# chenxuhao/GraphMiner

Hardware: AMD Instinct MI355X
Metric: million edges processed/sec + total match count (higher is better)
Workload: dtype int32 (vertex ids, offsets; uint64 counts); 1 GPU; tc: triangle counting, LiveJournal stand-in; graph=rmat_s22_ef10_seed42, nv=4194304, ne_sym=81171116, tasks=40585558, max_degree=777, parallelism=task-chunk round-robin x1, replicated CSR

## Files before the change

graphminer_amd/csrc/gm_launch.hip:

```cpp
#include "gm_launch.h"

using namespace gm;

__host__ __device__ static inline int finalize_math(int mode, unsigned long long base, const unsigned long long *c, unsigned long long *out) {
  if (mode == FIN_MOTIF3) {
    out[0] = c[2] - c[0];
    out[1] = c[1];
  } else if (mode == FIN_MOTIF3_FORMULA) {
    out[0] = base - 3ull * c[0];
    out[1] = c[0];
  } else if (mode == FIN_RAW4) {
    out[0] = c[0]; out[1] = c[1]; out[2] = c[2]; out[3] = c[3];
  } else if (mode == FIN_HALF_SIGNED) {
    out[0] = (unsigned long long)((long long)c[0] >> 1);
  } else {
    out[0] = c[0];
  }
  return mode == FIN_RAW4 ? 4 : (mode == FIN_MOTIF3 || mode == FIN_MOTIF3_FORMULA) ? 2 : 1;
}

__global__ void finalize_kernel(int mode, unsigned long long base, const unsigned long long *__restrict__ c,
                                unsigned long long *__restrict__ out) {
  if (threadIdx.x != 0 || blockIdx.x != 0) return;
  finalize_math(mode, base, c, out);
// ... 163 lines not shown
      if (const int rc_t = ensure_tasklists(g)) return rc_t;
    }
  }
  if (pl.support && !pl.sup_part && !pl.wtri && !g->diamond.sup) HIP_TRY(g->diamond.sup.alloc(sizeof(unsigned) * (size_t)std::max<long long>(g->ne, 1)));
  if (pl.support && !pl.sup_part && !pl.wtri && world == 1 && pl.use_tct && !pl.use_kst && !(la->tune[6] & GM_T6_SUP_ATOMICS)) {
    if (const int rc_m = ensure_sup_masks(g)) return rc_m;
    pl.sup_masks = g->sup_masks.built();
  }
  setup_trace("run_pattern: task lists");
  if (pl.split_stage) {
    RowFilter rb;
    rb.tct = (pl.use_kst && !pl.support && g->kst->skip_from < g->nv) ? 2 : 1;
    rb.only_lo = kStageCap;
    rb.only_hi = kTctStageMax;
    if (const int rc_b = get_table(g, pl.target, true, 0, pl.part_cap, kTctStageMax, &pl.tab_big, rb, kBitmapMinDeg)) return rc_b;
    if ((long long)pl.tab_big->n / world < 2ll * g->cu_count * 4 && !gm_opt("GM_TCT_SPLIT_ALWAYS")) {
      pl.tab_big = nullptr;
      pl.split_stage = false;
      pl.tct_stage = kTctStageMax;
    }
  }
  pl.corner_from = pl.use_kst ? g->kst->skip_from : (pl.use_tct ? g->tasklists->skip_from : 0x7fffffff);
  pl.tc_core = pl.use_tct && !pl.support && pl.corner_from < g->nv;
  pl.sup_core = pl.support && !pl.wtri && !pl.use_kst && pl.corner_from < g->nv;
  if (pl.sup_core) {
    if (const int rc_c = ensure_sup_corner(g)) return rc_c;
  }
  RowFilter rf;
  rf.tct = pl.use_tct ? ((pl.tc_core && pl.use_kst) ? 2 : 1) : 0;
  if (pl.tct_long) { rf.skip_lo = kTctStageMax; rf.skip_hi = 0x7fffffff; }
  if (pl.split_stage) { rf.skip_lo = kStageCap; rf.skip_hi = 0x7fffffff; }
  if (pl.use_wide) rf.only_lo = kCbMaxDeg;
  pl.cls_lo = kClassRowMin;
  if (const char *e = gm_sweep_env("GM_CLS_LO")) pl.cls_lo = std::max(64, atoi(e));
  pl.use_range = pl.use_classes && !(la->tune[6] & GM_T6_GIANT_SPLIT) && hrow_fits(g->nv, 2);
  if (pl.use_classes) { rf.skip_lo = pl.cls_lo; rf.skip_hi = pl.use_range ? 0x7fffffff : kStageCapBig; }
  if (int rc = get_table(g, pl.target, !pl.clique, pl.clique ? kBitWords : 0, pl.part_cap, pl.use_tct ? pl.tct_stage : stage_cap_of(pl.pat), &pl.tab, rf, pl.use_classes ? kStageCapBig : kBitmapMinDeg)) return rc;
  if (pl.tct_long && !pl.support) {
    RowFilter rl;
    rl.only_lo = kTctStageMax;
    if (int rc = get_table(g, pl.target, true, 0, kPartCostCap, kStageCap, &pl.tab_long, rl, kBitmapMinDeg)) return rc;
  }
  pl.tab_cls[0] = pl.tab;
  if (pl.use_classes) {
    RowFilter r1, r2;
    r1.only_lo = pl.cls_lo; r1.only_hi = kStageCapMid;
    r2.only_lo = kStageCapMid; r2.only_hi = kStageCapBig;
    unsigned long long cls_cap = (la->tune[6] & GM_T6_EAGER_PARTS) ? 4096ull
                                 : std::max<unsigned long long>(pl.part_cap, std::max<unsigned long long>((32ull << 20) / (unsigned long long)std::max(world, 1), 2ull << 20));
    if (const char *e = gm_sweep_env("GM_CLS_CAP_MKEYS")) cls_cap = (unsigned long long)std::max(1, atoi(e)) << 20;
    if (const char *e = gm_sweep_env("GM_CLS_CAP_KKEYS")) cls_cap = (unsigned long long)std::max(16, atoi(e)) << 10;
    if (int rc = get_table(g, 1, false, 0, cls_cap, kStageCapMid, &pl.tab_cls[1], r1, 0x7fffffff)) return rc;
    if (int rc = get_table(g, 1, false, 0, cls_cap, kStageCapBig, &pl.tab_cls[2], r2, 0x7fffffff)) return rc;
    if (pl.use_range) {
      RowFilter r3;
      r3.only_lo = kStageCapBig;
      int gtarget = kGiantEdges;
      {
        unsigned long long ge = 0;
        if (int rc = giant_task_edges(g, &ge)) return rc;
        const unsigned long long per = ge / ((unsigned long long)g->cu_count * (unsigned long long)giant_per_cu() * 4ull * (unsigned long long)world);
        gtarget = (int)std::max<unsigned long long>(512, std::min<unsigned long long>((unsigned long long)kGiantEdges, per));
        gtarget = (gtarget + 63) & ~63;
        if (const char *e = gm_sweep_env("GM_GIANT_TARGET")) gtarget = std::max(64, std::min(atoi(e), kGiantEdges));
      }
      if (int rc = get_table(g, gtarget, true, 0, 0ull, kStageCapBig, &pl.tab_cls[3], r3, 0x7fffffff)) return rc;
    }
  }
  if (pl.use_wide) {
    if (int rc = get_clique_plan(g, rank, world, la->policy, pl.target, pl.part_cap, &pl.plan)) return rc;
  }
  return GM_OK;
}

static int take_share(PatternRun &r, ChunkTable *tb, MineParams &q) {
  gm_graph *g = r.ctx.g;
  const gm_launch *la = &r.ctx.la;
  const PatternPlan &pl = r.pl;
  const int world = r.ctx.world, rank = r.ctx.rank;
  q.chunks = tb->d;
  q.chunk_slot = tb->d_slot;
  q.bitmaps = tb->d_bitmaps;
  q.bitmap_words = tb->bitmap_words;
  q.row_slot = tb->d_row_slot;
  const long long n = (long long)tb->n;
  long long first = 0, step = 1, count = 0;
  const bool clique_pat = pl.pat == PAT_CLIQUE4 || pl.pat == PAT_CLIQUEK;
  const int which = (((world > 1 && !pl.sym_pat) || clique_pat) ? 1 : 0) ^ ((la->tune[6] & GM_T6_SWAP_ORDERS) ? 1 : 0);
  const bool lpt = la->policy == GM_PART_ROUND_ROBIN && tb->d_order[which] && !(la->tune[6] & GM_T6_CHUNK_ID_ORDER);
  q.order = lpt ? tb->d_order[which] : nullptr;
  if (world > 1 && la->policy != GM_PART_VERTEX && tb->d_edges) {
    const ShareOrder *so = nullptr;
    if (int rcs = get_share_order(g, tb, world, rank, la->policy, lpt ? which : -1, &so)) return rcs;
    q.first = 0;
    q.step = 1;
    q.count = (int)so->n;
    q.order = so->d;
    r.my_edges += so->edges;
    return GM_OK;
  }
  if (la->policy == GM_PART_VERTEX) {
    if (int rcv = table_host_views(g, tb)) return rcv;
    chunk_range_of_vertex_share(tb, g->nv, rank, world, &first, &count);
  } else {
    gm_partition((int64_t)n, rank, world, la->policy, (int64_t *)&first, (int64_t *)&step, (int64_t *)&count);
  }
  q.first = (int)first;
  q.step = (int)step;
  q.count = (int)count;
  if (first == 0 && step == 1 && count == n) { r.my_edges += tb->total_edges; return GM_OK; }
  if (int rcv = table_host_views(g, tb)) return rcv;
  if (step == 1) r.my_edges += tb->edge_prefix[first + count] - tb->edge_prefix[first];
  else for (long long j = first; j < n; j += step) {
    const size_t c = lpt ? (size_t)tb->order[which][(size_t)j] : (size_t)j;
    r.my_edges += tb->edge_prefix[c + 1] - tb->edge_prefix[c];
  }
  return GM_OK;
}

static int fill_mine_params(PatternRun &r, int k) {
  gm_graph *g = r.ctx.g;
  const gm_launch *la = &r.ctx.la;
  const PatternPlan &pl = r.pl;
  MineParams &p = r.p;
  memset(&p, 0, sizeof p);
  p.g = graph_view(g);
  if (int rc = ensure_edesc(g)) return rc;
  p.g.edesc = *g->edesc;
  if (pl.use_tct) {
    const TaskLists &tl = *g->tasklists;
    const KeyStream &ks = *g->kst;
    p.g.trp = tl.trp;
    p.g.tdesc = tl.tdesc;
    p.g.tedge = pl.support ? tl.tedge.get() : nullptr;
    if (pl.sup_masks) {
      p.g.tmoff = g->sup_masks->tmoff;
      p.smask = g->sup_masks->smask;
    }
    if (pl.use_kst && pl.support) {
      const KeyEntries &k2 = *g->kst_entries;
      p.g.kst = k2.kst2 ? k2.kst2 : ks.kst;
      p.g.kst_rp = ks.rp;
      p.g.kst_et = k2.kst_et ? k2.kst_et : ks.kst_et;
      p.g.trp = ks.trpl;
      p.g.tdesc = k2.tdescl2 ? k2.tdescl2 : ks.tdescl;
      p.g.tedge = k2.tedgel ? k2.tedgel : ks.tedgel;
    } else if (pl.use_kst) {
      p.g.kst = ks.kst;
      p.g.kst_rp = ks.rp;
      p.g.trp = ks.trpl;
      p.g.tdesc = ks.tdescl;
    } else if (!pl.support && tl.colk && tl.tdesck && !(la->tune[6] & GM_T6_NO_KEYSTREAM)) {
      p.g.col = tl.colk;
      p.g.tdesc = tl.tdesck;
    }
  }
  if (int rc = take_share(r, pl.tab, p)) return rc;
  p.grab = la->tune[1] > 0 ? la->tune[1] : 1;
  if (la->tune[1] <= 0 && pl.use_tct && !pl.support && p.count >= 8ll * (long long)g->cu_count * (long long)(pl.tct_stage <= kStageCap ? 6 : 4)) p.grab = 2;
  p.cost_x_step = la->tune[2] > 0 ? la->tune[2] - 1 : 1;
  p.cost_y_step = la->tune[3] > 0 ? la->tune[3] - 1 : 6;
  p.cost_x_base = (la->tune[7] & 255) > 0 ? ((la->tune[7] >> 4) & 15) : 2;
  p.cost_y_base = (la->tune[7] & 255) > 0 ? (la->tune[7] & 15) : 2;
  p.cost_y_bitmap = la->tune[7] >> 8;
  p.k = k;
  p.flags = (la->tune[5] == 1) ? 1 : 0;
  p.flags |= (la->tune[6] & GM_T6_KERNEL_FLAGS_MASK) << 1;
  if (la->tune[6] & GM_T6_HROW_MUL32) p.flags |= 1 << 23;
  if (la->tune[6] & GM_T6_HSET_FALLBACK) p.flags |= 1 << 22;
  if (la->tune[6] & GM_T6_KCLIQUE_ANY_WIDTH) p.flags |= 1 << 20;
  p.counters = g->d_counters;
  p.queue = queue_word(g, QW_MAIN);
  return GM_OK;
}

static int prepare_scratch(PatternRun &r, int k) {
  gm_graph *g = r.ctx.g;
  const gm_launch *la = &r.ctx.la;
  const PatternPlan &pl = r.pl;
  MineParams &p = r.p;
  const size_t lds = mine_lds_bytes(pl.pat);
  r.per_cu = (int)std::max<size_t>(1, std::min<size_t>(8, (160 * 1024) / lds));
  if (la->tune[4] > 0) r.per_cu = la->tune[4];
  r.want = ((long long)p.count + (long long)p.grab - 1) / (long long)p.grab;
  r.grid = grid_for(r.want, g->cu_count, r.per_cu);
  if (pl.clique && pl.tab->max_bit_words > 0) {
    const unsigned long long region = pl.tab->max_bit_words + 4096ull;
    const int plist = (g->max_deg + 64) & ~63;
    const unsigned long long slot_words = (pl.pat == PAT_CLIQUEK) ? (unsigned long long)(k - 2) * (region + (unsigned long long)plist) : pl.tab->max_bit_words;
    p.scratch_region = region;
    p.scratch_plist = plist;
    {
      size_t free_b = 0, total_b = 0;
      (void)hipMemGetInfo(&free_b, &total_b);
      const unsigned long long budget = (unsigned long long)(free_b + g->scratch.bytes) / 2ull;
      const unsigned long long fit = budget / std::max<unsigned long long>(slot_words * sizeof(unsigned), 1ull);
      if (fit == 0) {
        g_last_error = "k-clique: the bit-matrix of the longest DAG row (" + std::to_string(g->max_deg) + " entries) does not fit the device memory";
        return GM_ERR_TOO_LARGE;
      }
      if ((unsigned long long)r.grid > fit) r.grid = (int)fit;
    }
    const size_t need = (size_t)slot_words * sizeof(unsigned) * (size_t)r.grid;
    if (int rc = ensure_scratch(g, need)) return rc;
    p.scratch = g->scratch.p;
    p.scratch_words = slot_words;
  }
  if (pl.use_wide && pl.plan && pl.plan->core_base >= 0 && gm_sweep_env("GM_CLIQUE_SIDE_STREAM")) {
    for (int i = 0; i < 2; ++i) {
      if (!g->aux_stream[i]) {
        HIP_TRY(hipStreamCreateWithFlags(&g->aux_stream[i], hipStreamNonBlocking));
        HIP_TRY(hipEventCreateWithFlags(&g->aux_done[i], hipEventDisableTiming));
      }
    }
  }
  if (pl.use_classes) {
    if (pl.tab_cls[3] && pl.tab_cls[3]->n > 0) {
      if (int rc = ensure_scratch(g, (size_t)giant_scratch_words(g->max_deg) * sizeof(unsigned) * (size_t)g->cu_count * (size_t)giant_per_cu())) return rc;
    }
  }
  return GM_OK;
}

#ifdef GM_DEBUG_CHUNKS
static int debug_chunks_begin(PatternRun &r) {
  ChunkTable *tab = r.pl.tab;
  HIP_TRY(r.debug_ticks.alloc(sizeof(unsigned long long) * std::max<size_t>(tab->n, 1)));
  HIP_TRY(hipMemset(r.debug_ticks, 0, sizeof(unsigned long long) * std::max<size_t>(tab->n, 1)));
  r.p.chunk_ticks = r.debug_ticks;
  return GM_OK;
}
static int debug_chunks_dump(PatternRun &run) {
  gm_graph *g = run.ctx.g;
  hipStream_t stream = run.ctx.stream;
  ChunkTable *tab = run.pl.tab;
  const MineParams &p = run.p;
  const Pattern pat = run.pl.pat;
  unsigned long long *d_ticks = p.chunk_ticks;
  HIP_TRY(hipStreamSynchronize(stream));
  std::vector<unsigned long long> ticks(tab->n);
  HIP_TRY(hipMemcpy(ticks.data(), d_ticks, sizeof(unsigned long long) * tab->n, hipMemcpyDeviceToHost));
  run.debug_ticks.reset();
  std::vector<ChunkRec> recs(tab->n);
  HIP_TRY(hipMemcpy(recs.data(), tab->d, sizeof(ChunkRec) * tab->n, hipMemcpyDeviceToHost));
  if (int rcv = table_host_views(g, tab)) return rcv;
  const std::vector<int> *h_rp_p = nullptr;
  if (int rcv = host_rp(g, &h_rp_p)) return rcv;
  const std::vector<int> &h_rp = *h_rp_p;
  std::vector<size_t> idx(tab->n);
  for (size_t i = 0; i < tab->n; ++i) idx[i] = i;
  std::sort(idx.begin(), idx.end(), [&](size_t a, size_t b) { return ticks[a] > ticks[b]; });
  unsigned long long tot = 0;
  for (auto t : ticks) tot += t;
  if (const char *dump = gm_sweep_env("GM_CHUNK_DUMP")) {
    static int dump_no = 0;
    const std::string name = std::string(dump) + "." + std::to_string(dump_no++) + ".pat" + std::to_string((int)pat);
    FILE *f = fopen(name.c_str(), "w");
    if (f) {
      fprintf(f, "pos,cid,rows,entries,rowlen,whole,part,nparts,cost,us\n");
      for (size_t pos = 0; pos < tab->n; ++pos) {
        const size_t cid = p.order ? (size_t)(p.order == tab->d_order[0] ? tab->order[0][pos] : tab->order[1][pos]) : pos;
        const ChunkRec &r = recs[cid];
        const bool whole = r.e_begin == h_rp[r.u_begin] && r.e_end == h_rp[r.u_end];
        fprintf(f, "%zu,%zu,%d,%d,%d,%d,%d,%d,%llu,%.1f\n", pos, cid, r.u_end - r.u_begin, r.e_end - r.e_begin,
                h_rp[r.u_begin + 1] - h_rp[r.u_begin], (int)whole, r.part, r.nparts, tab->cost[cid], ticks[pos] / 100.0);
      }
      fclose(f);
    }
  }
  fprintf(stderr, "[chunks] n=%zu total ticks %llu (100 MHz): mean %.1f us\n", tab->n, tot, tot / 100.0 / std::max<size_t>(tab->n, 1));
  for (size_t k = 0; k < std::min<size_t>(12, tab->n); ++k) {
    const size_t pos = idx[k];
    const size_t cid = p.order ? (size_t)(p.order == tab->d_order[0] ? tab->order[0][pos] : tab->order[1][pos]) : pos;
    const ChunkRec &r = recs[cid];
    fprintf(stderr, "[chunks] #%zu pos %zu: %.1f us  rows [%d,%d) entries [%d,%d) n=%d part %d/%d rowlen %d\n", k, pos, ticks[pos] / 100.0,
            r.u_begin, r.u_end, r.e_begin, r.e_end, r.e_end - r.e_begin, r.part, r.nparts, h_rp[r.u_begin + 1] - h_rp[r.u_begin]);
  }
  return GM_OK;
}
#endif

static int launch_clique4_rounds(PatternRun &r) {
  gm_graph *g = r.ctx.g;
  const gm_launch *la = &r.ctx.la;
  hipStream_t stream = r.ctx.stream;
  CliquePlan *plan = r.pl.plan;
  const MineParams &p = r.p;
  {
    ChunkTable *tn = plan->tabN;
    if (plan->n_count == (long long)tn->n) {
      r.my_edges += tn->total_edges;
    } else {
      if (int rc = table_host_views(g, tn)) return rc;
    }
    for (long long i = 0; i < plan->n_count && plan->n_count != (long long)tn->n; ++i) {
      const long long pos = plan->n_first + i * plan->n_step;
      const size_t c = plan->d_order ? (size_t)tn->order[plan->order_which][(size_t)pos] : (size_t)pos;
      r.my_edges += tn->edge_prefix[c + 1] - tn->edge_prefix[c];
    }
    r.my_edges += plan->wide_edges;
  }
  HIP_TRY(hipMemsetAsync(g->arena.queue, 0, 65536, stream));
  setup_trace("launch: clique prologue");
  const bool prof = gm_sweep_env("GM_WIDE_PROFILE") != nullptr;
  int qword = 0;
  for (const auto &rd : plan->rounds) {
// ... 730 lines not shown
```

graphminer_amd/csrc/gm_mine.h:

```cpp
#pragma once
#include <hip/hip_runtime.h>
#include <stdint.h>
#include <stdlib.h>

const char *gm_opt(const char *name);
inline const char *gm_sweep_env(const char *name) {
#ifdef GM_DEVEL
  return getenv(name);
#else
  (void)name;
  return nullptr;
#endif
}

namespace gm {

constexpr int kWavesPerBlock = 4;
constexpr int kStageCap = 1024;
#ifndef GM_STAGE_WIDE
#define GM_STAGE_WIDE 3072
#endif
constexpr int kStageCapWide = GM_STAGE_WIDE;
constexpr int kStageCapMid = 8191;
constexpr int kStageCapBig = 24576;
constexpr int kMaxChunkVerts = 256;
constexpr int kMarkWindow = 512;
#ifndef GM_TILES
#define GM_TILES 2
#endif
#define GM_TILES_DEFAULT GM_TILES
#ifndef GM_FILTER_LOG2
#define GM_FILTER_LOG2 15
#endif
constexpr int kFilterLog2 = GM_FILTER_LOG2;
constexpr int kFilterBits = 1 << kFilterLog2;
constexpr int kFilterWords = kFilterBits / 32;
constexpr int kQueueCap = 64 * (GM_TILES_DEFAULT + 1);
#ifndef GM_BIT_WORDS
#define GM_BIT_WORDS 2048
#endif
constexpr int kBitWords = GM_BIT_WORDS;
static_assert(GM_BIT_WORDS >= 2048 && GM_BIT_WORDS % 64 == 0, "rows of up to 2048 columns (stride 64) need 32 of them in one LDS group / tile");

constexpr int kSplitBatchMinKeys = 2048;
#ifndef GM_SPLIT_BATCH
#define GM_SPLIT_BATCH 16
#endif
constexpr int kSplitBatch = GM_SPLIT_BATCH;
struct ChunkRec {
  int u_begin, u_end, e_begin, e_end;
  int part, nparts;
  int batch, pad_;
};

struct GraphView {
  int nv;
  int ne;
  const int *rp;
  const int *col;
  const int2 *edesc = nullptr;
  const int *trp = nullptr;
  const int2 *tdesc = nullptr;
  const int *tedge = nullptr;
  const unsigned *tmoff = nullptr;
  const unsigned *kst = nullptr;
  const int *kst_rp = nullptr;
  const int2 *kst_et = nullptr;
};

#ifndef GM_LONG_LIST
#define GM_LONG_LIST 192
#endif
constexpr int kLongList = GM_LONG_LIST;
constexpr unsigned kNoMask = 0xffffffffu;
#ifndef GM_SUP_MASK_MIN_TAIL
#define GM_SUP_MASK_MIN_TAIL 2
#endif
constexpr int kSupMaskMinTail = GM_SUP_MASK_MIN_TAIL;
constexpr int kSupMaskSpare = 3;

enum Pattern : int { PAT_TC = 0, PAT_DIAMOND = 1, PAT_MOTIF3 = 2, PAT_CLIQUE4 = 3, PAT_CLIQUEK = 4 ,
                     PAT_MOTIF4E = 5 ,
                     PAT_DAGSTATS = 6 ,
                     PAT_SUPPORT = 7 ,
                     PAT_SUPPORT_PART = 8 ,
                     PAT_CLIQUEK_DEEP = 9 ,
                     PAT_WTRI = 10  };

#ifndef GM_PROBE_COST
#define GM_PROBE_COST 1
#endif
constexpr int kProbeCost = GM_PROBE_COST;
#ifndef GM_MID_PROBE_COST
#define GM_MID_PROBE_COST 1
#endif
constexpr int kMidProbeCost = GM_MID_PROBE_COST;
constexpr int kMidRowMax = 16384;
__host__ __device__ inline bool sym_hosts(int a, int b, int u, int v, int stage_cap) {
  const bool u_longer = (a > b) || (a == b && u > v);
  const int dl = u_longer ? a : b, ds = u_longer ? b : a;
  const int k = (dl <= kMidRowMax) ? kMidProbeCost : kProbeCost;
  const bool shorter_hosts = dl > stage_cap && ds <= stage_cap && (long long)dl < (long long)k * ds;
  return u_longer != shorter_hosts;
}

constexpr int kStageCapClique = 1024;
constexpr int stage_cap_of(int pat) {
  return (pat == PAT_DIAMOND || pat == PAT_MOTIF3 || pat == PAT_MOTIF4E) ? kStageCapWide
         : (pat == PAT_CLIQUE4 || pat == PAT_CLIQUEK || pat == PAT_CLIQUEK_DEEP) ? kStageCapClique : kStageCap;
}

struct MineParams {
  GraphView g;
  const ChunkRec *chunks;
  const int *chunk_slot;
  const int *order;
  unsigned long long *chunk_ticks;
  const unsigned *bitmaps;
  unsigned long long bitmap_words;
  const int *row_slot;
  int first, step, count;
  int grab;
  unsigned *queue;
  unsigned long long *counters;
  unsigned *scratch;
  unsigned long long scratch_words;
  unsigned long long scratch_region;
  int scratch_plist;
  int cost_x_step;
  int cost_y_step;
  int cost_x_base;
  int cost_y_base;
  int cost_y_bitmap;
  int k;
  unsigned long long *smask;
  int flags;
};

enum SglPattern : int { SGL_RECTANGLE = 0, SGL_HOUSE = 1, SGL_PENTAGON = 2, SGL_DIAMOND = 3  };

struct SglParams {
  GraphView g;
  long long first, step, count;
  int chunk;
  unsigned *queue;
  unsigned long long *counters;
  int *scratch;
  int max_deg;
};
hipError_t launch_sgl_nested(int pat, const SglParams &p, int grid_blocks, hipStream_t stream);

struct RectParams {
  GraphView g;
  const int *idx0;
  const unsigned long long *block_prefix;
  unsigned long long first, step, count;
  unsigned long long nblocks;
  int group;
  unsigned long long *queue;
  unsigned long long *counters;
};
hipError_t launch_rect_flat(const RectParams &p, bool pentagon, int grid_blocks, hipStream_t stream);
hipError_t launch_idx0(const GraphView &g, int *idx0, hipStream_t stream);

struct RectAccParams {
  GraphView g;
  const int *idx0;
  const int4 *tasks;
  unsigned long long first, step, count;
  unsigned *acc;
  int *touched;
  unsigned long long acc_stride;
  unsigned long long *queue;
  unsigned long long *counters;
  unsigned long long n_cut;
  int cut;
  const int *bnd0;
  int bnd_stride;
};
hipError_t launch_rect_acc(const RectAccParams &p, int grid_blocks, hipStream_t stream);

#ifndef GM_RECT_LDS_WORDS
#define GM_RECT_LDS_WORDS 32768
#endif
constexpr int kRectLdsWords = GM_RECT_LDS_WORDS;
constexpr int kRectLdsRanges = 32;
constexpr int kRectLdsWaves = 16;
struct RectLdsRanges {
  int n;
  int rb[kRectLdsRanges + 1];
  int lb[kRectLdsRanges];
};
struct RectLdsParams {
  GraphView g;
  const int *idx0;
  const int2 *tasks;
  unsigned long long first, step, count;
  const int *bnd;
  RectLdsRanges r;
  unsigned long long *queue;
  unsigned long long *counters;
};
hipError_t launch_rect_lds(const RectLdsParams &p, int grid_blocks, hipStream_t stream);
hipError_t launch_rect_bounds(const GraphView &g, const RectLdsRanges &r, int *bnd, hipStream_t stream);
hipError_t launch_rect_blockmax(const GraphView &g, int *blockmax, hipStream_t stream);
hipError_t launch_rect_work_cut(const GraphView &g, const int *idx0, const int *bnd0, int bnd_stride, unsigned long long *work, hipStream_t stream);
hipError_t launch_rect_work(const GraphView &g, const int *idx0, unsigned long long *work, hipStream_t stream);

struct HouseAccParams {
  GraphView g;
  const unsigned *t;
  const unsigned *tlt;
  const int4 *tasks;
  unsigned long long first, step, count;
  unsigned long long *acc;
  int *touched;
  unsigned long long acc_stride;
  unsigned long long *queue;
  unsigned long long *counters;
  unsigned long long n_cut;
// ... 393 lines not shown
```

graphminer_amd/csrc/gm_tch.hip:

```cpp
#include <type_traits>
#include "gm_flat.h"

namespace gm {

#ifndef GM_TCH_TILES
#define GM_TCH_TILES 4
#endif
constexpr int kTchTiles = GM_TCH_TILES;
#ifndef GM_TCH_TILES_SMALL
#define GM_TCH_TILES_SMALL 2
#endif
constexpr int kTchTilesSmall = GM_TCH_TILES_SMALL;
constexpr int kTchFlatTilesSmall = 4, kTchFlatTilesBig = 8;

#ifndef GM_TCH_LONG_LIST
#define GM_TCH_LONG_LIST 384
#endif
constexpr int kTchLongList = GM_TCH_LONG_LIST;

constexpr int kTchOvfCap = 128;
constexpr unsigned kTchEmpty = 0xffffffffu, kTchMarker = 0xfffffffeu;
constexpr unsigned kTchMul = 0x9E3779B1u;

template <int BITWIN>
struct alignas(16) TchWave {
  int2 desc[GM_WAVE];
  unsigned bits[BITWIN / 32 + 8];
};

#ifndef GM_TCH_WAVES_BIG
#define GM_TCH_WAVES_BIG 4
#endif
#ifndef GM_TCH_MIN_WG_BIG
#define GM_TCH_MIN_WG_BIG 4
#endif
template <int STAGE>
constexpr int tch_waves() { return STAGE <= 1024 ? kWavesPerBlock : GM_TCH_WAVES_BIG; }
template <int STAGE>
struct alignas(16) TchLds {
  uint4 table[STAGE];
  int rpl[kMaxChunkVerts + 1];
  int trpl[kMaxChunkVerts + 1];
  static constexpr int kBitWindow = STAGE <= 1024 ? 8192 : 4096;
  TchWave<kBitWindow> w[tch_waves<STAGE>()];
  int ovf_key[kTchOvfCap];
  int ovf_salt[kTchOvfCap];
  int n_ovf;
  int next_batch;
  unsigned queue_pos;
  int next_group;
};
static_assert(kTchOvfCap == 2 * GM_WAVE, "the surplus list is scanned two entries per lane");

template <int STAGE>
struct TchHash {
  static constexpr int LB = STAGE == 1024 ? 10 : 11;
  static_assert((1 << LB) == STAGE, "one bucket per stage entry");
  static constexpr unsigned kMask = (unsigned)(STAGE - 1) << 4;
  static __device__ __forceinline__ unsigned bucket(int x, unsigned s) { return ((((unsigned)x * kTchMul) >> (28 - LB)) & kMask) ^ s; }
  static __device__ __forceinline__ unsigned salt(int local_row) { return (((unsigned)local_row * 37u) & (unsigned)(STAGE - 1)) << 4; }
  static __device__ __forceinline__ int row_of(unsigned s) { return (int)(((s >> 4) * 941u) & (unsigned)(STAGE - 1)); }
};

__device__ __forceinline__ int tch_local_row(const int *rpl, const int nvl, const int e) {
  int lo = 0, hi = nvl - 1;
  while (lo < hi) {
    const int mid = (lo + hi + 1) >> 1;
    if (rpl[mid] <= e) lo = mid; else hi = mid - 1;
  }
  return lo;
}

template <int STAGE, int T>
__device__ __forceinline__ void tch_probe(const TchLds<STAGE> &B, const int *__restrict__ col, const bool fallback, const int (&key)[T],
                                          const unsigned (&salt)[T], const unsigned long long (&inm)[T], unsigned long long (&hm)[T],
                                          unsigned long long (&nm)[T]) {
  if (fallback) {
#pragma unroll
    for (int q = 0; q < T; ++q) {
      bool f = false;
      if (__builtin_amdgcn_inverse_ballot_w64(inm[q])) {
        const int lo = TchHash<STAGE>::row_of(salt[q]);
        const int rs = B.rpl[lo], rn = B.rpl[lo + 1] - rs;
        const int pos = lower_bound(col + rs, rn, key[q]);
        f = pos < rn && col[rs + pos] == key[q];
      }
      hm[q] = __ballot(f);
      nm[q] = 0ull;
    }
    return;
  }
  uint4 w[T];
#pragma unroll
  for (int q = 0; q < T; ++q)
    w[q] = *reinterpret_cast<const uint4 *>(reinterpret_cast<const char *>(B.table) + TchHash<STAGE>::bucket(key[q], salt[q]));
#pragma unroll
  for (int q = 0; q < T; ++q) {
    const unsigned k = (unsigned)key[q];
    const unsigned long long m = __ballot(w[q].x == k) | __ballot(w[q].y == k) | __ballot(w[q].z == k) | __ballot(w[q].w == k);
    hm[q] = m & inm[q];
    nm[q] = __ballot(w[q].w == kTchMarker) & ~m & inm[q];
  }
}

template <int STAGE, int T>
__device__ __forceinline__ unsigned tch_surplus(const TchLds<STAGE> &B, const int lane, const int (&key)[T], const unsigned (&salt)[T],
                                                const unsigned long long (&nm)[T]) {
  const int k0 = B.ovf_key[lane], k1 = B.ovf_key[lane + GM_WAVE];
  const int s0 = B.ovf_salt[lane], s1 = B.ovf_salt[lane + GM_WAVE];
  unsigned c = 0;
#pragma unroll
  for (int q = 0; q < T; ++q) {
    unsigned long long rest = nm[q];
    while (rest) {
      const int src = __ffsll((long long)rest) - 1;
      rest &= rest - 1;
      const int k = readlane(key[q], src), s = readlane((int)salt[q], src);
      if (__ballot(((k0 == k) & (s0 == s)) | ((k1 == k) & (s1 == s))) != 0ull) ++c;
    }
  }
  return c;
}

template <int STAGE>
__device__ __forceinline__ unsigned tch_pass(TchLds<STAGE> &B, TchWave<TchLds<STAGE>::kBitWindow> &L, const int *__restrict__ col, const bool fallback, const int lane,
                                             const int llen_all, const int key_base, const unsigned salt_l) {
  constexpr int T = STAGE <= 1024 ? kTchTilesSmall : kTchTiles;
  constexpr int TF = STAGE <= 1024 ? kTchFlatTilesSmall : kTchFlatTilesBig;
  unsigned cnt = 0;
  if (wave_max_nonneg(llen_all) == 0) return 0u;
  const bool is_long = llen_all >= kTchLongList;
  const int llen = is_long ? 0 : llen_all;

  unsigned long long lm = __ballot(is_long);
  while (lm) {
    const int src = __ffsll((long long)lm) - 1;
    lm &= lm - 1;
    const int base = readlane(key_base, src);
    const int n = readlane(llen_all, src);
    const unsigned s_u = (unsigned)readlane((int)salt_l, src);
    const int *__restrict__ kp = col + base;
    auto process = [&](auto kc, const int (&key)[T], const unsigned long long (&inm)[T]) {
      constexpr int K = decltype(kc)::value;
      int k2[K];
      unsigned salt[K];
      unsigned long long i2[K], hm[K], nm[K];
#pragma unroll
      for (int q = 0; q < K; ++q) {
        k2[q] = key[q];
        salt[q] = s_u;
        i2[q] = inm[q];
      }
      tch_probe<STAGE, K>(B, col, fallback, k2, salt, i2, hm, nm);
      unsigned long long any_need = 0ull;
#pragma unroll
      for (int q = 0; q < K; ++q) {
        cnt += (unsigned)__popcll(hm[q]);
        any_need |= nm[q];
      }
      if (any_need != 0ull) cnt += tch_surplus<STAGE, K>(B, lane, k2, salt, nm);
    };
    constexpr int G = GM_WAVE * T;
    int nxt[T];
#pragma unroll
    for (int q = 0; q < T; ++q) nxt[q] = kp[min(q * GM_WAVE + lane, n - 1)];
    int t = 0;
    for (; t + 2 * G <= n; t += G) {
      int key[T];
      unsigned long long inm[T];
#pragma unroll
      for (int q = 0; q < T; ++q) {
        key[q] = nxt[q];
        inm[q] = ~0ull;
      }
      const int *__restrict__ kn = kp + (t + G);
#pragma unroll
      for (int q = 0; q < T; ++q) nxt[q] = kn[(unsigned)(q * GM_WAVE + lane)];
      process(std::integral_constant<int, T>{}, key, inm);
    }
    for (; t < n; t += G) {
      int key[T];
      unsigned long long inm[T];
#pragma unroll
      for (int q = 0; q < T; ++q) {
        key[q] = nxt[q];
        inm[q] = __ballot((t + q * GM_WAVE + lane) < n);
      }
#pragma unroll
      for (int q = 0; q < T; ++q) nxt[q] = kp[min(t + G + q * GM_WAVE + lane, n - 1)];
      const int tiles = min(T, (n - t + GM_WAVE - 1) >> 6);
      if (tiles >= T) process(std::integral_constant<int, T>{}, key, inm);
      else if (tiles == 1) process(std::integral_constant<int, 1>{}, key, inm);
      else if constexpr (T > 2) {
        if (tiles == 2) process(std::integral_constant<int, 2>{}, key, inm);
        else process(std::integral_constant<int, (T > 2 ? 3 : 1)>{}, key, inm);
      }
    }
  }

  const int incl = wave_incl_scan_add(llen);
  const int total = readlane(incl, GM_WAVE - 1);
  if (total == 0) return cnt;
  const int off = incl - llen;
  const unsigned long long nzm = __ballot(llen > 0);
  if (llen > 0) L.desc[rank_below(nzm)] = make_int2(key_base - off, (int)salt_l);
  constexpr int G = GM_WAVE * TF, kBitWin = TchLds<STAGE>::kBitWindow;
  constexpr int TH = 4, NH = TF / TH;
  static_assert(TF % TH == 0, "tile groups are made of half-groups of four");
  struct Grp {
    int key[NH][TH];
    unsigned salt[NH][TH];
    unsigned long long inm[NH][TH];
  };
  for (int wb = 0; wb < total; wb += kBitWin) {
    const int wn = min(kBitWin, total - wb);
    const int nw = ((wn + G - 1) / G) * (G / 32) + 2;
    for (int i = lane; i < nw; i += GM_WAVE) L.bits[i] = 0u;
    wave_sync();
    if (llen > 0 && off > wb && off < wb + kBitWin) atomicOr(&L.bits[(off - 1 - wb) >> 5], 1u << ((off - 1 - wb) & 31));
    int carry = __popcll(__ballot(llen > 0 && off <= wb)) - 1;
    wave_sync();
    auto stage_a = [&](const int g, Grp &r) {
      int2 d[TF];
      bool in[TF];
      const int mw = (int)L.bits[((g * G) >> 5) + (lane & (2 * TF - 1))];
#pragma unroll
      for (int q = 0; q < TF; ++q) {
        const unsigned long long m = ((unsigned long long)(unsigned)readlane(mw, 2 * q + 1) << 32) | (unsigned)readlane(mw, 2 * q);
        const int own = carry + rank_below(m);
        carry += __popcll(m);
        in[q] = (wb + g * G + q * GM_WAVE + lane) < total;
        r.inm[q / TH][q % TH] = __ballot(in[q]);
        d[q] = L.desc[in[q] ? own : 0];
      }
#pragma unroll
      for (int q = 0; q < TF; ++q) {
        r.key[q / TH][q % TH] = col[in[q] ? d[q].x + (wb + g * G + q * GM_WAVE + lane) : 0];
        r.salt[q / TH][q % TH] = (unsigned)d[q].y;
      }
    };
    auto stage_b = [&](const Grp &r) {
#pragma unroll
      for (int h = 0; h < NH; ++h) {
        unsigned long long hm[TH], nm[TH];
        tch_probe<STAGE, TH>(B, col, fallback, r.key[h], r.salt[h], r.inm[h], hm, nm);
        unsigned long long any_need = 0ull;
#pragma unroll
        for (int q = 0; q < TH; ++q) {
          cnt += (unsigned)__popcll(hm[q]);
          any_need |= nm[q];
        }
        if (any_need != 0ull) cnt += tch_surplus<STAGE, TH>(B, lane, r.key[h], r.salt[h], nm);
      }
    };
    const int ng = (wn + G - 1) / G;
    Grp cur;
    stage_a(0, cur);
    for (int g = 0; g + 1 < ng; ++g) {
      Grp nxt;
      stage_a(g + 1, nxt);
      stage_b(cur);
      cur = nxt;
    }
    stage_b(cur);
    wave_sync();
  }
  return cnt;
}

#ifndef GM_TCH_MIN_WG
#define GM_TCH_MIN_WG 6
#endif
template <int STAGE>
__global__ __launch_bounds__((tch_waves<STAGE>() * GM_WAVE), (STAGE <= 1024 ? GM_TCH_MIN_WG : GM_TCH_MIN_WG_BIG))
void tch_kernel(const MineParams p) {
  __shared__ TchLds<STAGE> B;
  using H = TchHash<STAGE>;
  const int lane = threadIdx.x & (GM_WAVE - 1);
  const int wave = threadIdx.x >> 6;
  constexpr int nthreads = tch_waves<STAGE>() * GM_WAVE;
  const int tid = threadIdx.x;
  const int *__restrict__ rp = p.g.rp;
  const int *__restrict__ col = p.g.col;
  const int *__restrict__ trp = p.g.trp;
  const int2 *__restrict__ tdesc = p.g.tdesc;
  auto &L = B.w[wave];
  unsigned long long c0 = 0;
  for (;;) {
    if (tid == 0) B.queue_pos = atomicAdd(p.queue, (unsigned)p.grab);
    __syncthreads();
    const unsigned q = B.queue_pos;
    if (q >= (unsigned)p.count) break;
    const unsigned qe = min(q + (unsigned)p.grab, (unsigned)p.count);
    constexpr int kU = 4;
    auto chunk_at = [&](const unsigned ci) {
      const size_t pos = (size_t)p.first + (size_t)ci * (size_t)p.step;
      return p.chunks[p.order ? (size_t)p.order[pos] : pos];
    };
    ChunkRec rn = chunk_at(q);
    bool have_pre = false;
    int xn[kU], rpn = 0, trpn = 0;
    for (unsigned ci = q; ci < qe; ++ci) {
      const ChunkRec r = rn;
      const int ub = r.u_begin, nvl = r.u_end - r.u_begin;
      const int eb = r.e_begin, nel = r.e_end - r.e_begin;
      unsigned *fill32 = reinterpret_cast<unsigned *>(&B.w[0]);
      if (have_pre) {
        if (tid <= nvl) {
          B.rpl[tid] = rpn;
          B.trpl[tid] = trpn;
        }
        for (int i = tid + nthreads; i <= nvl; i += nthreads) {
          B.rpl[i] = rp[ub + i];
          B.trpl[i] = trp[ub + i];
        }
      } else {
        for (int i = tid; i <= nvl; i += nthreads) {
          B.rpl[i] = rp[ub + i];
          B.trpl[i] = trp[ub + i];
        }
      }
      {
        const uint4 empty = make_uint4(kTchEmpty, kTchEmpty, kTchEmpty, kTchEmpty);
        for (int i = tid; i < STAGE; i += nthreads) B.table[i] = empty;
        for (int i = tid; i < STAGE / 2; i += nthreads) fill32[i] = 0u;
        if (tid < kTchOvfCap) {
          B.ovf_key[tid] = -1;
          B.ovf_salt[tid] = -1;
        }
        if (tid == 0) {
          B.n_ovf = 0;
          B.next_batch = 0;
          B.next_group = 0;
        }
      }
      __syncthreads();
      unsigned *slots = reinterpret_cast<unsigned *>(B.table);
      for (int i0 = tid; i0 < nel; i0 += kU * nthreads) {
        int x[kU];
        if (have_pre && i0 == tid) {
#pragma unroll
          for (int j = 0; j < kU; ++j) x[j] = xn[j];
        } else {
#pragma unroll
          for (int j = 0; j < kU; ++j) x[j] = col[eb + min(i0 + j * nthreads, nel - 1)];
        }
#pragma unroll
        for (int j = 0; j < kU; ++j) {
          const int i = i0 + j * nthreads;
          if (i < nel) {
            const unsigned s = H::salt(tch_local_row(B.rpl, nvl, eb + i));
            const unsigned b = H::bucket(x[j], s) >> 4;
            const unsigned shift = (b & 1u) * 16u;
            const unsigned slot = (atomicAdd(&fill32[b >> 1], 1u << shift) >> shift) & 0xffffu;
            if (slot < 4u) {
              slots[(b << 2) + slot] = (unsigned)x[j];
            } else {
              const int jo = atomicAdd(&B.n_ovf, 1);
              if (jo < kTchOvfCap) {
                B.ovf_key[jo] = x[j];
                B.ovf_salt[jo] = (int)s;
              }
            }
          }
        }
      }
      __syncthreads();
      for (int b = tid; b < STAGE; b += nthreads) {
        const unsigned c = (fill32[b >> 1] >> ((b & 1) * 16)) & 0xffffu;
        if (c > 4u) {
          const unsigned x3 = slots[(b << 2) + 3];
          const int jo = atomicAdd(&B.n_ovf, 1);
          if (jo < kTchOvfCap) {
            B.ovf_key[jo] = (int)x3;
            B.ovf_salt[jo] = (int)(H::bucket((int)x3, 0u) ^ ((unsigned)b << 4));
          }
          slots[(b << 2) + 3] = kTchMarker;
        }
      }
      __syncthreads();
      const bool fallback = B.n_ovf > kTchOvfCap || (p.flags & (1 << 22)) != 0;
      have_pre = ci + 1 < qe;
      if (have_pre) {
        rn = chunk_at(ci + 1);
        const int nel_n = rn.e_end - rn.e_begin, nvl_n = rn.u_end - rn.u_begin;
#pragma unroll
        for (int j = 0; j < kU; ++j) xn[j] = col[rn.e_begin + min(tid + j * nthreads, max(nel_n - 1, 0))];
        rpn = rp[rn.u_begin + min(tid, nvl_n)];
        trpn = trp[rn.u_begin + min(tid, nvl_n)];
      }
      if (p.g.kst != nullptr) {
        constexpr int TS = 4, GS = TS * GM_WAVE;
        const int kb = p.g.kst_rp[ub], kn = p.g.kst_rp[ub + nvl] - kb;
        const unsigned *__restrict__ kp = p.g.kst + kb;
        auto grab = [&]() {
          int gi = 0;
          if (lane == 0) gi = atomicAdd(&B.next_group, 1);
          return (readfirst(gi) * r.nparts + r.part) * GS;
        };
        unsigned nxt[TS];
        int g0 = kn > 0 ? grab() : 0;
        if (g0 < kn) {
#pragma unroll
          for (int q = 0; q < TS; ++q) nxt[q] = kp[min(g0 + q * GM_WAVE + lane, kn - 1)];
        }
        while (g0 < kn) {
          const int gc = g0;
          int key[TS];
          unsigned salt[TS];
          unsigned long long inm[TS], hm[TS], nm[TS];
#pragma unroll
          for (int q = 0; q < TS; ++q) {
            key[q] = (int)(nxt[q] & 0xffffffu);
            salt[q] = H::salt((int)(((nxt[q] >> 24) - (unsigned)ub) & 255u));
            inm[q] = __ballot(gc + q * GM_WAVE + lane < kn);
          }
          g0 = grab();
          if (g0 < kn) {
#pragma unroll
            for (int q = 0; q < TS; ++q) nxt[q] = kp[min(g0 + q * GM_WAVE + lane, kn - 1)];
          }
          tch_probe<STAGE, TS>(B, col, fallback, key, salt, inm, hm, nm);
          unsigned long long any_need = 0ull;
          unsigned cnt = 0;
#pragma unroll
          for (int q = 0; q < TS; ++q) {
            cnt += (unsigned)__popcll(hm[q]);
            any_need |= nm[q];
          }
          if (any_need != 0ull) cnt += tch_surplus<STAGE, TS>(B, lane, key, salt, nm);
          c0 += (unsigned long long)cnt;
        }
      }
      const int tb = B.trpl[0], ntask = B.trpl[nvl] - tb;
      for (;;) {
        int bi = 0;
        if (lane == 0) bi = atomicAdd(&B.next_batch, 1);
        bi = readfirst(bi) * r.nparts + r.part;
        const int t0 = bi * GM_WAVE;
        if (t0 >= ntask) break;
        const bool valid = t0 + lane < ntask;
        const int te = tb + min(t0 + lane, ntask - 1);
        const int2 d = tdesc[te];
        const int lo = tch_local_row(B.trpl, nvl, te);
        const int ru = B.rpl[lo], a = B.rpl[lo + 1] - ru;
        const bool act = valid && d.y > 0 && a > 0;
        c0 += (unsigned long long)tch_pass<STAGE>(B, L, col, fallback, lane, act ? d.y : 0, d.x, H::salt(lo));
      }
      __syncthreads();
    }
  }
  if (lane == 0 && c0) atomicAdd(&p.counters[0], c0);
}

int tch_per_cu(int stage) {
  if (stage <= 1024) return 6;
  return (int)std::max<size_t>(1, std::min<size_t>(163840 / sizeof(TchLds<kTctStageMax>), 2048 / (tch_waves<kTctStageMax>() * GM_WAVE)));
}
hipError_t launch_tch(const MineParams &p, int stage, int grid_blocks, hipStream_t stream) {
  static_assert(sizeof(TchLds<1024>) * 6 <= 163840, "six workgroups per CU");
  static_assert(sizeof(TchLds<kTctStageMax>) <= 163840, "one workgroup per CU at least");
  static_assert(sizeof(TchWave<4096>) * tch_waves<kTctStageMax>() >= (size_t)kTctStageMax * 2, "fill counters alias the wave scratch");
  if (p.g.trp == nullptr || p.g.tdesc == nullptr) return hipErrorInvalidValue;
  const dim3 grid((unsigned)grid_blocks);
  if (stage <= 1024) hipLaunchKernelGGL((tch_kernel<1024>), grid, dim3(kWavesPerBlock * GM_WAVE), 0, stream, p);
  else hipLaunchKernelGGL((tch_kernel<kTctStageMax>), grid, dim3(tch_waves<kTctStageMax>() * GM_WAVE), 0, stream, p);
  return hipGetLastError();
}

}

__global__ void gm_touch_tch_kernel() {}
void gm_touch_tch() { hipLaunchKernelGGL(gm_touch_tch_kernel, dim3(1), dim3(1), 0, 0); }
```

Measured before the change: 25750 Medges/s.

## Use pre-scaled biased byte offsets for flat key gathers in triangle hash pass

Adds a narrow addressing mode for the flattened key-probe loop in the triangle-count hash kernel. Descriptor bases are stored pre-shifted to byte offsets, and the column gather uses a biased 32-bit offset added to a scalar base, so address arithmetic stays 32-bit. A wide fallback is kept for graphs whose key array is too large, chosen on the host. It also splits full tile groups from the guarded tail so full groups skip per-lane bounds checks, and reads the descriptor LDS through a raw address-space pointer. The cost is two kernel instantiations and reliance on offset-overflow reasoning.

```diff
diff --git a/graphminer_amd/csrc/gm_launch.hip b/graphminer_amd/csrc/gm_launch.hip
--- a/graphminer_amd/csrc/gm_launch.hip
+++ b/graphminer_amd/csrc/gm_launch.hip
@@ -339,6 +339,7 @@
       p.g.tdesc = ks.tdescl;
     } else if (!pl.support && tl.colk && tl.tdesck && !(la->tune[6] & GM_T6_NO_KEYSTREAM)) {
       p.g.col = tl.colk;
+      p.g.col_entries = (long long)g->ne + (long long)tl.n_copy_keys;
       p.g.tdesc = tl.tdesck;
     }
   }
diff --git a/graphminer_amd/csrc/gm_mine.h b/graphminer_amd/csrc/gm_mine.h
--- a/graphminer_amd/csrc/gm_mine.h
+++ b/graphminer_amd/csrc/gm_mine.h
@@ -66,6 +66,7 @@
   const unsigned *kst = nullptr;
   const int *kst_rp = nullptr;
   const int2 *kst_et = nullptr;
+  long long col_entries = 0;
 };
 
 #ifndef GM_LONG_LIST
diff --git a/graphminer_amd/csrc/gm_tch.hip b/graphminer_amd/csrc/gm_tch.hip
--- a/graphminer_amd/csrc/gm_tch.hip
+++ b/graphminer_amd/csrc/gm_tch.hip
@@ -1,5 +1,6 @@
 #include <type_traits>
 #include "gm_flat.h"
+#include "gm_tch_rule.h"
 
 namespace gm {
 
@@ -17,6 +18,7 @@
 #define GM_TCH_LONG_LIST 384
 #endif
 constexpr int kTchLongList = GM_TCH_LONG_LIST;
+
 
 constexpr int kTchOvfCap = 128;
 constexpr unsigned kTchEmpty = 0xffffffffu, kTchMarker = 0xfffffffeu;
@@ -122,7 +124,7 @@
   return c;
 }
 
-template <int STAGE>
+template <int STAGE, bool WIDE>
 __device__ __forceinline__ unsigned tch_pass(TchLds<STAGE> &B, TchWave<TchLds<STAGE>::kBitWindow> &L, const int *__restrict__ col, const bool fallback, const int lane,
                                              const int llen_all, const int key_base, const unsigned salt_l) {
   constexpr int T = STAGE <= 1024 ? kTchTilesSmall : kTchTiles;
@@ -203,47 +205,66 @@
   if (total == 0) return cnt;
   const int off = incl - llen;
   const unsigned long long nzm = __ballot(llen > 0);
-  if (llen > 0) L.desc[rank_below(nzm)] = make_int2(key_base - off, (int)salt_l);
+  if (llen > 0) L.desc[rank_below(nzm)] = make_int2(WIDE ? key_base - off : (int)((unsigned)(key_base - off) << 2), (int)salt_l);
   constexpr int G = GM_WAVE * TF, kBitWin = TchLds<STAGE>::kBitWindow;
   constexpr int TH = 4, NH = TF / TH;
   static_assert(TF % TH == 0, "tile groups are made of half-groups of four");
+  static_assert(kTchFlatBias >= 4u * (unsigned)(GM_WAVE * (kTchLongList - 1) + G), "the bias covers every flattened position of a batch and the over-run of its last group");
   struct Grp {
     int key[NH][TH];
     unsigned salt[NH][TH];
     unsigned long long inm[NH][TH];
   };
+  using LdsDesc = const __attribute__((address_space(3))) unsigned long long;
+  const unsigned dbase = (unsigned)readfirst((int)(unsigned)(size_t)(LdsDesc *)reinterpret_cast<const unsigned long long *>(&L.desc[0]));
+  const char *const colb = reinterpret_cast<const char *>(col) - kTchFlatBias;
+  const unsigned lane4 = ((unsigned)lane << 2) + kTchFlatBias;
   for (int wb = 0; wb < total; wb += kBitWin) {
     const int wn = min(kBitWin, total - wb);
     const int nw = ((wn + G - 1) / G) * (G / 32) + 2;
     for (int i = lane; i < nw; i += GM_WAVE) L.bits[i] = 0u;
     wave_sync();
     if (llen > 0 && off > wb && off < wb + kBitWin) atomicOr(&L.bits[(off - 1 - wb) >> 5], 1u << ((off - 1 - wb) & 31));
-    int carry = __popcll(__ballot(llen > 0 && off <= wb)) - 1;
+    unsigned carry = dbase + ((unsigned)(__popcll(__ballot(llen > 0 && off <= wb)) - 1) << 3);
     wave_sync();
-    auto stage_a = [&](const int g, Grp &r) {
+    auto stage_a = [&](auto full, const int g, Grp &r) {
+      constexpr bool FULL = decltype(full)::value;
       int2 d[TF];
       bool in[TF];
+      const int p0 = wb + g * G;
       const int mw = (int)L.bits[((g * G) >> 5) + (lane & (2 * TF - 1))];
 #pragma unroll
       for (int q = 0; q < TF; ++q) {
         const unsigned long long m = ((unsigned long long)(unsigned)readlane(mw, 2 * q + 1) << 32) | (unsigned)readlane(mw, 2 * q);
-        const int own = carry + rank_below(m);
-        carry += __popcll(m);
-        in[q] = (wb + g * G + q * GM_WAVE + lane) < total;
-        r.inm[q / TH][q % TH] = __ballot(in[q]);
-        d[q] = L.desc[in[q] ? own : 0];
+        const unsigned own = carry + ((unsigned)rank_below(m) << 3);
+        carry += (unsigned)__popcll(m) << 3;
+        asm volatile("" : "+s"(carry));
+        in[q] = FULL || (p0 + q * GM_WAVE + lane) < total;
+        r.inm[q / TH][q % TH] = FULL ? ~0ull : __ballot(in[q]);
+        const unsigned long long dw = *(LdsDesc *)(size_t)(in[q] ? own : dbase);
+        d[q] = make_int2((int)(unsigned)dw, (int)(unsigned)(dw >> 32));
       }
 #pragma unroll
       for (int q = 0; q < TF; ++q) {
-        r.key[q / TH][q % TH] = col[in[q] ? d[q].x + (wb + g * G + q * GM_WAVE + lane) : 0];
+        if constexpr (WIDE) {
+          const unsigned idx = (unsigned)d[q].x + (unsigned)(p0 + q * GM_WAVE + lane);
+          r.key[q / TH][q % TH] = col[in[q] ? idx : 0u];
+        } else {
+          const unsigned idle = kTchFlatBias - ((unsigned)(p0 + q * GM_WAVE) << 2);
+          const unsigned voff = in[q] ? (unsigned)d[q].x + lane4 : idle;
+          r.key[q / TH][q % TH] = *reinterpret_cast<const int *>(colb + ((size_t)(unsigned)p0 << 2) + (size_t)voff + (size_t)(q * GM_WAVE * 4));
+        }
         r.salt[q / TH][q % TH] = (unsigned)d[q].y;
       }
     };
-    auto stage_b = [&](const Grp &r) {
+    auto stage_b = [&](auto full, const Grp &r) {
+      constexpr bool FULL = decltype(full)::value;
 #pragma unroll
       for (int h = 0; h < NH; ++h) {
-        unsigned long long hm[TH], nm[TH];
-        tch_probe<STAGE, TH>(B, col, fallback, r.key[h], r.salt[h], r.inm[h], hm, nm);
+        unsigned long long inm[TH], hm[TH], nm[TH];
+#pragma unroll
+        for (int q = 0; q < TH; ++q) inm[q] = FULL ? ~0ull : r.inm[h][q];
+        tch_probe<STAGE, TH>(B, col, fallback, r.key[h], r.salt[h], inm, hm, nm);
         unsigned long long any_need = 0ull;
 #pragma unroll
         for (int q = 0; q < TH; ++q) {
@@ -253,16 +274,28 @@
         if (any_need != 0ull) cnt += tch_surplus<STAGE, TH>(B, lane, r.key[h], r.salt[h], nm);
       }
     };
-    const int ng = (wn + G - 1) / G;
+    constexpr std::true_type kFull{};
+    constexpr std::false_type kGuarded{};
+    const int nfull = wn / G, ng = (wn + G - 1) / G;
     Grp cur;
-    stage_a(0, cur);
-    for (int g = 0; g + 1 < ng; ++g) {
-      Grp nxt;
-      stage_a(g + 1, nxt);
-      stage_b(cur);
-      cur = nxt;
+    if (nfull == 0) {
+      stage_a(kGuarded, 0, cur);
+    } else {
+      stage_a(kFull, 0, cur);
+      for (int g = 0; g + 1 < nfull; ++g) {
+        Grp nxt;
+        stage_a(kFull, g + 1, nxt);
+        stage_b(kFull, cur);
+        cur = nxt;
+      }
+      if (ng > nfull) {
+        Grp nxt;
+        stage_a(kGuarded, nfull, nxt);
+        stage_b(kFull, cur);
+        cur = nxt;
+      }
     }
-    stage_b(cur);
+    stage_b(kGuarded, cur);
     wave_sync();
   }
   return cnt;
@@ -271,7 +304,7 @@
 #ifndef GM_TCH_MIN_WG
 #define GM_TCH_MIN_WG 6
 #endif
-template <int STAGE>
+template <int STAGE, bool WIDE>
 __global__ __launch_bounds__((tch_waves<STAGE>() * GM_WAVE), (STAGE <= 1024 ? GM_TCH_MIN_WG : GM_TCH_MIN_WG_BIG))
 void tch_kernel(const MineParams p) {
   __shared__ TchLds<STAGE> B;
@@ -321,17 +354,19 @@
         }
       }
       {
-        const uint4 empty = make_uint4(kTchEmpty, kTchEmpty, kTchEmpty, kTchEmpty);
+        unsigned ones = kTchEmpty, zero = 0u;
+        asm volatile("" : "+v"(ones), "+v"(zero));
+        const uint4 empty = make_uint4(ones, ones, ones, ones);
         for (int i = tid; i < STAGE; i += nthreads) B.table[i] = empty;
-        for (int i = tid; i < STAGE / 2; i += nthreads) fill32[i] = 0u;
+        for (int i = tid; i < STAGE / 2; i += nthreads) fill32[i] = zero;
         if (tid < kTchOvfCap) {
-          B.ovf_key[tid] = -1;
-          B.ovf_salt[tid] = -1;
+          B.ovf_key[tid] = (int)ones;
+          B.ovf_salt[tid] = (int)ones;
         }
         if (tid == 0) {
-          B.n_ovf = 0;
-          B.next_batch = 0;
-          B.next_group = 0;
+          B.n_ovf = (int)zero;
+          B.next_batch = (int)zero;
+          B.next_group = (int)zero;
         }
       }
       __syncthreads();
@@ -432,7 +467,7 @@
           c0 += (unsigned long long)cnt;
         }
       }
-      const int tb = B.trpl[0], ntask = B.trpl[nvl] - tb;
+      const int tb = readfirst(B.trpl[0]), ntask = readfirst(B.trpl[nvl]) - tb;
       for (;;) {
         int bi = 0;
         if (lane == 0) bi = atomicAdd(&B.next_batch, 1);
@@ -445,7 +480,7 @@
         const int lo = tch_local_row(B.trpl, nvl, te);
         const int ru = B.rpl[lo], a = B.rpl[lo + 1] - ru;
         const bool act = valid && d.y > 0 && a > 0;
-        c0 += (unsigned long long)tch_pass<STAGE>(B, L, col, fallback, lane, act ? d.y : 0, d.x, H::salt(lo));
+        c0 += (unsigned long long)tch_pass<STAGE, WIDE>(B, L, col, fallback, lane, act ? d.y : 0, d.x, H::salt(lo));
       }
       __syncthreads();
     }
@@ -463,8 +498,15 @@
   static_assert(sizeof(TchWave<4096>) * tch_waves<kTctStageMax>() >= (size_t)kTctStageMax * 2, "fill counters alias the wave scratch");
   if (p.g.trp == nullptr || p.g.tdesc == nullptr) return hipErrorInvalidValue;
   const dim3 grid((unsigned)grid_blocks);
-  if (stage <= 1024) hipLaunchKernelGGL((tch_kernel<1024>), grid, dim3(kWavesPerBlock * GM_WAVE), 0, stream, p);
-  else hipLaunchKernelGGL((tch_kernel<kTctStageMax>), grid, dim3(tch_waves<kTctStageMax>() * GM_WAVE), 0, stream, p);
+  const bool wide = tch_wide_form(tch_key_entries(p.g.ne, p.g.col_entries), gm_opt("GM_TCH_WIDE_NE"));
+  const dim3 block_small(kWavesPerBlock * GM_WAVE), block_big(tch_waves<kTctStageMax>() * GM_WAVE);
+  if (stage <= 1024) {
+    if (wide) hipLaunchKernelGGL((tch_kernel<1024, true>), grid, block_small, 0, stream, p);
+    else hipLaunchKernelGGL((tch_kernel<1024, false>), grid, block_small, 0, stream, p);
+  } else {
+    if (wide) hipLaunchKernelGGL((tch_kernel<kTctStageMax, true>), grid, block_big, 0, stream, p);
+    else hipLaunchKernelGGL((tch_kernel<kTctStageMax, false>), grid, block_big, 0, stream, p);
+  }
   return hipGetLastError();
 }
 
diff --git a/graphminer_amd/csrc/gm_tch_rule.h b/graphminer_amd/csrc/gm_tch_rule.h
--- /dev/null
+++ b/graphminer_amd/csrc/gm_tch_rule.h
@@ -0,0 +1,21 @@
+#pragma once
+#include <stdlib.h>
+
+namespace gm {
+
+constexpr unsigned kTchFlatBias = 1u << 17;
+constexpr long long kTchNarrowEntries = (1ll << 30) - (long long)(kTchFlatBias >> 2) - 64;
+
+inline long long tch_key_entries(long long ne, long long col_entries) { return col_entries > ne ? col_entries : ne; }
+
+inline bool tch_wide_form(long long key_entries, const char *option) {
+  long long wide_from = kTchNarrowEntries;
+  if (option) {
+    long long v = atoll(option);
+    if (v < 0) v = 0;
+    if (v < wide_from) wide_from = v;
+  }
+  return key_entries >= wide_from;
+}
+
+}
```

After: 27000 Medges/s, median of 6. 4.8% higher.
